# fplll/fplll

Hardware: AMD Instinct MI355X
Metric: enum nodes/sec (BKZ-60 SVP enumeration, dim-180 q-ary lattice) (higher is better)
Workload: dtype f64; 1 GPU; BASELINE configs[2]: beta=60 blocks kappa=0,1,2 of the 180-dim q-ary lattice, one Enumeration::enumerate call per step, radius min(0.99 r,1.1 GH), FastEvaluator(1); pruning=LinearPruningParams(60,30), counting_rule=fplll (after the bound test), summed in 64 bit

## Files before the change

### fplll_amd/build.py

```python
import os
import subprocess
import sys

HERE = os.path.dirname(os.path.abspath(__file__))
ROOT = os.path.dirname(HERE)
CSRC = os.path.join(HERE, "csrc")
LIBDIR = os.path.join(HERE, "lib")

HIP_SOURCES = ["enum_kernel.hip", "enum_walk.hip", "enum_kernel_cvp.hip", "enum_walk_cvp.hip", "enum_deal.hip", "enum_order.hip", "enum_host.hip", "gso_kernel.hip", "gso_sweep2.hip", "lll_kernel.hip", "lll_kernel_early.hip", "hlll_kernel.hip", "hh_blocked.hip", "hh_rows.hip", "hlll_x.hip", "lll_x.hip", "bkz_kernel.hip", "bkzs_kernel.hip", "bkz_kernel_u.hip", "bkzs_kernel_u.hip", "gso_host.hip", "pruner_volume.hip", "pruner_search.hip", "gso_util_host.hip"]
HIP_HEADERS = ["dev_mem.h", "dev_cache.h", "trace.h", "pruner_tables.h", "pruner_engine.h", "enum_device.h", "enum_order.h", "enum_wave.h", "gso_device.h", "gso_wave.h", "gso_sweep2.h", "ftx.h", "lll_wave.h", "lll_stream.h", os.path.join(ROOT, "include", "fplll_hip.h")]
HIPCC_FLAGS = [
    "--offload-arch=gfx950", "-O3", "-std=c++17",
    "-ffp-contract=off",
    "-fPIC", "-Wno-unused-value", "-Wno-inline-asm",
]


PER_FILE_FLAGS = {
    "enum_kernel.hip": ["-mllvm", "-structurizecfg-skip-uniform-regions=1", "-Xclang", "-disable-lifetime-markers"],
    "enum_walk.hip": ["-mllvm", "-structurizecfg-skip-uniform-regions=1", "-Xclang", "-disable-lifetime-markers"],
    "enum_kernel_cvp.hip": ["-mllvm", "-structurizecfg-skip-uniform-regions=1", "-Xclang", "-disable-lifetime-markers"],
    "enum_walk_cvp.hip": ["-mllvm", "-structurizecfg-skip-uniform-regions=1", "-Xclang", "-disable-lifetime-markers"],
    "bkzs_kernel.hip": ["-mllvm", "-structurizecfg-skip-uniform-regions=1", "-Xclang", "-disable-lifetime-markers"],
    "bkzs_kernel_u.hip": ["-mllvm", "-structurizecfg-skip-uniform-regions=1", "-Xclang", "-disable-lifetime-markers"],
    "bkz_kernel_u.hip": ["-mllvm", "-structurizecfg-skip-uniform-regions=1"],
    "lll_kernel.hip": ["-mllvm", "-structurizecfg-skip-uniform-regions=1"],
    "lll_kernel_early.hip": ["-mllvm", "-structurizecfg-skip-uniform-regions=1"],
    "bkz_kernel.hip": ["-mllvm", "-structurizecfg-skip-uniform-regions=1"],
    "hlll_kernel.hip": ["-mllvm", "-structurizecfg-skip-uniform-regions=1"],
    "gso_kernel.hip": ["-mllvm", "-structurizecfg-skip-uniform-regions=1"],
}


EXTRA_DEPS = {"lll_kernel_early.hip": ["lll_kernel.hip"], "enum_kernel_cvp.hip": ["enum_kernel.hip"],
              "enum_walk_cvp.hip": ["enum_walk.hip"], "bkz_kernel_u.hip": ["bkz_kernel.hip"],
              "bkzs_kernel_u.hip": ["bkzs_kernel.hip"]}


def _newer(target, deps):
    if not os.path.exists(target):
        return True
    t = os.path.getmtime(target)
    return any(os.path.exists(d) and os.path.getmtime(d) > t for d in deps)


def _run(cmd, cwd=None):
    print("[build]", " ".join(cmd), flush=True)
    subprocess.check_call(cmd, cwd=cwd)


def hipcc():
    for c in ("hipcc", "/opt/rocm/bin/hipcc"):
        try:
            subprocess.check_output([c, "--version"], stderr=subprocess.STDOUT)
            return c
        except Exception:
            continue
    raise RuntimeError("hipcc not found")


def build_hip(force=False):
    os.makedirs(LIBDIR, exist_ok=True)
    out = os.path.join(LIBDIR, "libfplll_hip.so")
    srcs = [os.path.join(CSRC, s) for s in HIP_SOURCES if os.path.exists(os.path.join(CSRC, s))]
    hdrs = [h if os.path.isabs(h) else os.path.join(CSRC, h) for h in HIP_HEADERS]
    extra = []
    if os.environ.get("FPHIP_GSO_RING"):
        extra.append("-DFPHIP_GSO_RING=" + os.environ["FPHIP_GSO_RING"])
        force = True
    objdir = os.path.join(LIBDIR, "obj")
    os.makedirs(objdir, exist_ok=True)
    objs = []
    relink = force or not os.path.exists(out)
    jobs = []
    for src in srcs:
        obj = os.path.join(objdir, os.path.basename(src) + ".o")
        objs.append(obj)
        more = [os.path.join(CSRC, x) for x in EXTRA_DEPS.get(os.path.basename(src), [])]
        if force or _newer(obj, [src, os.path.abspath(__file__)] + hdrs + more):
            jobs.append([hipcc()] + HIPCC_FLAGS + extra + PER_FILE_FLAGS.get(os.path.basename(src), []) +
                        ["-c", "-o", obj, src])
            relink = True
    if jobs:
        from concurrent.futures import ThreadPoolExecutor
        with ThreadPoolExecutor(max_workers=max(1, min(len(jobs), os.cpu_count() or 1))) as ex:
            list(ex.map(_run, jobs))
    if relink:
        _run([hipcc(), "--offload-arch=gfx950", "-fPIC", "-shared", "-pthread", "-o", out] + objs)
    return out


def build_shim(force=False):
    out = os.path.join(LIBDIR, "libfplll_hip_extenum.so")
    src = os.path.join(CSRC, "extenum_shim.cpp")
    if force or _newer(out, [src, os.path.join(ROOT, "include", "fplll_hip.h")]):
        _run(["g++", "-std=c++11", "-O2", "-fPIC", "-shared", "-o", out, src, "-L" + LIBDIR,
              "-lfplll_hip", "-Wl,-rpath,$ORIGIN", "-pthread"])
    return out


REF_HEADERS = "/root/reference"
CONDA = "/opt/conda"


def build_gso_dropin(force=False):
    out = os.path.join(LIBDIR, "libfplll_hip_gso.so")
    src = os.path.join(CSRC, "dropin", "matgso_hip.cpp")
    src2 = os.path.join(CSRC, "dropin", "mathouseholder_hip.cpp")
    hdr = os.path.join(CSRC, "dropin", "matgso_hip.h")
    hdr2 = os.path.join(CSRC, "dropin", "mathouseholder_hip.h")
    if not os.path.isdir(os.path.join(REF_HEADERS, "fplll")):
        return out if os.path.exists(out) else None
    if force or _newer(out, [src, src2, hdr, hdr2, os.path.join(ROOT, "include", "fplll_hip.h")]):
        cfg = os.path.join(LIBDIR, "obj", "fplll_cfg", "fplll")
        os.makedirs(cfg, exist_ok=True)
        with open(os.path.join(cfg, "fplll_config.h"), "w") as f:
            f.write("#ifndef FPLLL_CONFIG__H\n#define FPLLL_CONFIG__H\n#define FPLLL_MAJOR_VERSION 5\n"
                    "#define FPLLL_MINOR_VERSION 5\n#define FPLLL_MICRO_VERSION 0\n#define FPLLL_VERSION 5.5.0\n"
# ... 29 lines not shown
```

### fplll_amd/csrc/enum_host.hip

```cpp

#include <hip/hip_runtime.h>

#include <algorithm>
#include <chrono>
#include <cmath>
#include <cstdarg>
#include <cstdio>
#include <cstdlib>
#include <cstring>
#include <vector>

#include "../../include/fplll_hip.h"
#include "dev_mem.h"
#include "trace.h"
#include "enum_device.h"
#include "enum_order.h"


namespace fphip
{
template <bool MU_LDS, bool SUBS, bool DUAL>
__global__ void enum_phase_kernel(DevShared *g, HostCtl *h, TaskBuf in, TaskBuf out, int d,
                                  int Lmax, int stop, unsigned task_lo, unsigned task_hi,
                                  const unsigned *idxlist, int launch_idx, int count_nodes,
                                  unsigned budget, const double *xhi_root, double *gstk, int Tsplit,
                                  unsigned *qh, const unsigned *rcnt, unsigned rcap,
                                  unsigned long long bound_init);
template <int NQT, bool SUBS, bool DUAL>
__global__ void enum_top_kernel(DevShared *g, HostCtl *h, TopBuf in, unsigned n_in, TopBuf out_top,
                                int stop, TaskBuf out, double *xhi_root, int d, double maxdist,
                                int count_nodes, int launch_idx, double *gtop);
__global__ void task_key_kernel(TaskBuf in, unsigned n, int d, unsigned long long *keys,
                                const double *xhi_root, const unsigned *slots);
template <bool MU_LDS, bool DUAL, bool CHAIN>
__global__ void enum_walk_kernel(DevShared *g, HostCtl *h, TaskBuf in, TaskBuf out, int d, int Lmax, unsigned task_lo,
                                 unsigned task_hi, const unsigned *idxlist, int launch_idx, int count_nodes,
                                 unsigned budget, const double *xhi_root, double *gstk, int Tsplit, unsigned *qh,
                                 const unsigned *rcnt, unsigned rcap, unsigned long long bound_init);
template <bool MU_LDS, bool SUBS, bool DUAL>
__global__ void enum_phase_cvp_kernel(DevShared *g, HostCtl *h, TaskBuf in, TaskBuf out, int d, int Lmax, int stop,
                                      unsigned task_lo, unsigned task_hi, const unsigned *idxlist, int launch_idx,
                                      int count_nodes, unsigned budget, const double *xhi_root, double *gstk, int Tsplit,
                                      unsigned *qh, const unsigned *rcnt, unsigned rcap, unsigned long long bound_init);
template <bool MU_LDS, bool DUAL, bool CHAIN>
__global__ void enum_walk_cvp_kernel(DevShared *g, HostCtl *h, TaskBuf in, TaskBuf out, int d, int Lmax, unsigned task_lo,
                                     unsigned task_hi, const unsigned *idxlist, int launch_idx, int count_nodes,
                                     unsigned budget, const double *xhi_root, double *gstk, int Tsplit, unsigned *qh,
                                     const unsigned *rcnt, unsigned rcap, unsigned long long bound_init);
template <bool DUAL>
__global__ void enum_bfs_cvp_kernel(DevShared *g, double maxdist, QueueMem *qm, TaskBuf f0, TaskBuf f1, TaskBuf fin, int L0,
                                    int nlev, int floor_level, float heavy, int count_nodes, int compact_n, int shard_index,
                                    int shard_count);
size_t deal_work_bytes(unsigned n);
unsigned deal_tasks_device(hipStream_t s, const unsigned long long *keys, const double *pd, const unsigned *slot_of,
                           unsigned n, unsigned W, unsigned rank, unsigned *mine, void *work, size_t work_bytes);
size_t order_work_bytes(unsigned n);
int order_tasks_device(hipStream_t s, const DevShared *g, TaskBuf in, unsigned n, int d, const unsigned *slots,
                       unsigned *list, void *work, size_t work_bytes, int num_cus, int *sort_passes);
__global__ void task_pack_kernel(TaskBuf in, unsigned lo, unsigned n, double *rec, const double *xhi_root, int xstr);
__global__ void task_unpack_kernel(TaskBuf out, unsigned lo, unsigned n, const double *rec, double *xhi_root, int xstr,
                                   unsigned root_base);
template <bool DUAL>
__global__ void enum_bfs_kernel(DevShared *g, double maxdist, QueueMem *qm, TaskBuf f0, TaskBuf f1,
                                TaskBuf fin, int L0, int nlev, int floor_level, float heavy, int count_nodes,
                                int compact_n, int shard_index, int shard_count);
__global__ void enum_bfs_epilogue(const DevShared *g, HostCtl *h, const QueueMem *qm, unsigned rcap,
                                  unsigned *slots, double *pdc, const double *pd)
{
  __shared__ unsigned base[FPHIP_NQ + 1];
  if (threadIdx.x == 0)
  {
    unsigned tot = 0;
    for (int q = 0; q < FPHIP_NQ; ++q)
    {
      base[q] = tot;
      const unsigned c = qm->fin[q * FPHIP_QS];
      tot += c < rcap ? c : rcap;
    }
    base[FPHIP_NQ] = tot;
    h->pad[0]      = tot;
    h->pad[1]      = g->error_flags;
    __threadfence_system();
  }
  __syncthreads();
  if (slots)
    for (int q = 0; q < FPHIP_NQ; ++q)
      for (unsigned i = threadIdx.x; i < base[q + 1] - base[q]; i += blockDim.x)
      {
        slots[base[q] + i] = (unsigned)q * rcap + i;
        pdc[base[q] + i]   = pd[(size_t)q * rcap + i];
      }
}
}
using namespace fphip;

#include <mutex>
#include <vector>
namespace
{
struct PinnedBuf
{
  void *p;
  size_t bytes;
  bool busy;
};
std::mutex g_pinned_mutex;
std::vector<PinnedBuf> g_pinned;
}
#include "dev_cache.h"

void *fphip_pinned_get(size_t bytes)
{
  std::lock_guard<std::mutex> lk(g_pinned_mutex);
  PinnedBuf *best = nullptr;
  for (PinnedBuf &b : g_pinned)
    if (!b.busy && b.bytes >= bytes && (!best || b.bytes < best->bytes))
      best = &b;
  if (best)
  {
    best->busy = true;
    return best->p;
// ... 793 lines not shown
      fphip_dev_free(ctx->xhi_root, ctx->stream);
      ctx->xhi_root = nullptr;
      ctx->xhi_row  = 64;
      HIPCHK(ctx, fphip_dev_alloc((void **)&ctx->xhi_root, (size_t)ctx->cap * 192 * sizeof(double), ctx->stream));
      HIPCHK(ctx, hipMemsetAsync(ctx->xhi_root, 0, 192 * sizeof(double), ctx->stream));
      ctx->xhi_row = 192;
    }
    int cut = 64;
    for (int k = d - 1; k > 64; --k)
      if (logN[k] - logN[d] >= std::log(2048.0))
      {
        cut = k;
        break;
      }
    const int top_count = (o.shard_index == 0) ? 1 : 0;
    auto top_launch = [&](int in_idx, unsigned n_in, int stop, unsigned grid) -> int
    {
      HIPCHK(ctx, hipEventRecord(ctx->ev[0], ctx->stream));
#define FPHIP_TOP_LAUNCH(N, S_, D_)                                                                                \
  hipLaunchKernelGGL((enum_top_kernel<N, S_, D_>), dim3(grid), dim3(64), tlds, ctx->stream, ctx->g, ctx->h,          \
                     ctx->top[in_idx], n_in, ctx->top[in_idx ^ 1], stop, top_out, ctx->xhi_root, d, maxdist,        \
                     top_count, launch_idx, ctx->gtop)
      if (wide)
      {
        if (dual)
          FPHIP_TOP_LAUNCH(4, false, true);
        else if (subs)
          FPHIP_TOP_LAUNCH(4, true, false);
        else
          FPHIP_TOP_LAUNCH(4, false, false);
      }
      else if (dual)
        FPHIP_TOP_LAUNCH(2, false, true);
      else if (subs)
        FPHIP_TOP_LAUNCH(2, true, false);
      else
        FPHIP_TOP_LAUNCH(2, false, false);
#undef FPHIP_TOP_LAUNCH
      HIPCHK(ctx, hipGetLastError());
      HIPCHK(ctx, hipEventRecord(ctx->ev[1], ctx->stream));
      uint64_t nsub = 0;
      int rcw       = wait_serving(ctx, d, cb, subcb, user, &nsub);
      if (rcw != FPHIP_OK)
        return rcw;
      float tms = 0;
      HIPCHK(ctx, hipEventElapsedTime(&tms, ctx->ev[0], ctx->ev[1]));
      top_ms += tms;
      ++launch_idx;
      return FPHIP_OK;
    };
    int rct = top_launch(0, 1u, cut, 1u);
    if (rct != FPHIP_OK)
      return rct;
    if (cut > 64)
    {
      unsigned c1 = 0;
      HIPCHK(ctx, hipMemcpy(&c1, ctx->top[1].count, 4, hipMemcpyDeviceToHost));
      if (c1 > cap2)
      {
        snprintf(ctx->err, sizeof ctx->err, "more than %u top tasks: the block stays on the CPU enumerator", cap2);
        return FPHIP_UNSUPPORTED;
      }
      if (c1 > 0)
      {
        const unsigned per_cu = wide ? 4u : (unsigned)std::max<size_t>(1, (160 * 1024) / std::max<size_t>(tlds, 1));
        const unsigned grid   = std::min<unsigned>(c1, (unsigned)ctx->num_cus * std::min(per_cu, wide ? 4u : 8u));
        rct                   = top_launch(1, c1, 64, grid);
        if (rct != FPHIP_OK)
          return rct;
      }
    }
    HIPCHK(ctx, hipMemcpy(&top_tasks, ctx->buf[cur].count, 4, hipMemcpyDeviceToHost));
    if (top_tasks > top_out.cap)
    {
      snprintf(ctx->err, sizeof ctx->err,
               "more than %u surviving nodes at level 64: the block stays on the CPU enumerator", top_out.cap);
      return FPHIP_UNSUPPORTED;
    }
  }

  const int debug     = env_int("FPHIP_DEBUG", 0);
  const bool walk2    = env_int("FPHIP_WALK2", 1) != 0;
  const bool walk3    = env_int("FPHIP_WALK3", 1) != 0;
  uint64_t nsol       = 0;
  double kernel_ms    = top_ms, final_ms = 0.0;
  int launches        = 0;
  int L               = d > 64 ? 64 : d;
  unsigned C          = d > 64 ? top_tasks : 1;
  int final_tasks     = 0, final_L = d;
  const int max_split = env_int("FPHIP_MAX_SPLIT_PHASES", 6);
  double est_nodes = 0;
  for (int k = 0; k < d; ++k)
    est_nodes += std::exp(std::min(logN[k], 60.0));
  unsigned budget       = (unsigned)env_int("FPHIP_BUDGET", 1 << 22);
  const int max_rounds  = env_int("FPHIP_MAX_ROUNDS", 24);
  if (debug)
    fprintf(stderr, "[fphip] d=%d est_nodes=%.3e budget=%u\n", d, est_nodes, budget);
  unsigned long long moved_tasks = 0;
  unsigned xhi_used = d > 64 ? top_tasks : 0;
  bool in_final       = false;
  int round           = 0;
  unsigned prevC      = 0;

  bool regioned = false;
  unsigned n_slots = 0;
  bool bfs_sharded = false;
  if (use_bfs && C > 0)
  {
    FPHIP_RANGE("enum: breadth-first stage");
    const int L0        = L;
    const unsigned rcap = ctx->cap / FPHIP_NQ;
    const double want_tasks = o.target_tasks > 0 ? o.target_tasks : env_int("FPHIP_BFS_TASKS", 65536);
    float heavy = (float)std::max((double)env_int("FPHIP_BFS_HEAVY", 1024), est_nodes / want_tasks);
    int Lend = 1;
    for (int Lv = L0 - 1; Lv >= 1; --Lv)
      if (bfs_est0[Lv] <= heavy)
      {
        Lend = Lv;
        break;
      }
    Lend = std::max(Lend, std::min(L0 - 1, env_int("FPHIP_BFS_FLOOR", 4)));
    const int cnt_bfs = (o.shard_index == 0) ? 1 : 0;
    const bool shard_bfs = o.shard_count > 1 && d <= 64 && o.exchange && env_int("FPHIP_BFS_SHARD", 0) != 0;
    int n_single = 0;
    for (int Lv = L0; Lv > Lend; --Lv)
    {
      const double est_parents = (Lv == L0 ? (double)C : std::exp(std::min(logN[Lv] - logN[L0], 40.0)) * C);
      if (est_parents > env_int("FPHIP_BFS_SINGLE_MAX", 256))
        break;
      ++n_single;
    }
    HIPCHK(ctx, hipEventRecord(ctx->ev[0], ctx->stream));
    int Lv = L0, par = 0;
    int compact_n = (int)C;
    auto bfs_launch = [&](int nlev, unsigned grid, unsigned threads)
    {
      const TaskBuf &fa = ctx->buf[1 + par], &fb = ctx->buf[2 - par];
      const bool filter = shard_bfs && grid > 1u && !bfs_sharded;
      const int smode   = filter ? 1 : ((shard_bfs && !bfs_sharded) ? 2 : 0);
      const int scount  = smode ? o.shard_count * 4 + smode : 0;
      const int cnt     = (bfs_sharded || filter) ? 1 : cnt_bfs;
      if (filter)
        bfs_sharded = true;
      if (cvp)
        hipLaunchKernelGGL((enum_bfs_cvp_kernel<false>), dim3(grid), dim3(threads), 0, ctx->stream, ctx->g, maxdist,
                           ctx->qm, fa, fb, ctx->buf[0], Lv, nlev, Lend, heavy, cnt, compact_n, o.shard_index, scount);
      else if (dual)
        hipLaunchKernelGGL((enum_bfs_kernel<true>), dim3(grid), dim3(threads), 0, ctx->stream, ctx->g, maxdist,
                           ctx->qm, fa, fb, ctx->buf[0], Lv, nlev, Lend, heavy, cnt, compact_n, o.shard_index, scount);
      else
        hipLaunchKernelGGL((enum_bfs_kernel<false>), dim3(grid), dim3(threads), 0, ctx->stream, ctx->g, maxdist,
                           ctx->qm, fa, fb, ctx->buf[0], Lv, nlev, Lend, heavy, cnt, compact_n, o.shard_index, scount);
      Lv -= nlev;
      par ^= nlev & 1;
      compact_n = -1;
      ++launches;
    };
    if (n_single > 0)
      bfs_launch(n_single, 1u, 1024u);
    const unsigned bgrid = std::max(32u, ((unsigned)ctx->num_cus * (unsigned)env_int("FPHIP_BFS_WG_PER_CU", 1)) / 32u * 32u);
    while (Lv > Lend)
      bfs_launch(1, bgrid, 256u);
    const bool want_slots = (o.shard_count > 1 && !bfs_sharded) || ordered;
    hipLaunchKernelGGL(enum_bfs_epilogue, dim3(1), dim3(1024), 0, ctx->stream, ctx->g, ctx->h, ctx->qm, rcap,
                       want_slots ? ctx->slots : nullptr, want_slots ? ctx->pdc : nullptr, ctx->buf[0].pd);
    HIPCHK(ctx, hipGetLastError());
// ... 192 lines not shown
        task_x.resize((size_t)span * 64);
        task_level.resize(span);
        HIPCHK(ctx, hipMemcpy(task_x.data(), ctx->buf[cur].x, (size_t)span * 64 * sizeof(double), hipMemcpyDeviceToHost));
        HIPCHK(ctx, hipMemcpy(task_level.data(), ctx->buf[cur].level, (size_t)span * sizeof(int), hipMemcpyDeviceToHost));
        std::vector<unsigned> ranks((size_t)C * d);
        for (unsigned i = 0; i < C; ++i)
          order_vector(d, mut, rdiag, &task_x[(size_t)where[i] * 64], task_level[where[i]], &ranks[(size_t)i * d], nullptr);
        std::vector<unsigned> perm(C);
        for (unsigned i = 0; i < C; ++i)
          perm[i] = i;
        std::stable_sort(perm.begin(), perm.end(), [&](unsigned a, unsigned b)
                         { return order_before(d, &ranks[(size_t)a * d], &ranks[(size_t)b * d]); });
        for (unsigned i = 0; i < C; ++i)
          order_host[i] = where[perm[i]];
        HIPCHK(ctx, hipMemcpy(ctx->idxlist, order_host.data(), (size_t)C * 4, hipMemcpyHostToDevice));
        order_passes = -1;
      }
      else
        HIPCHK(ctx, hipMemcpy(order_host.data(), ctx->idxlist, (size_t)C * 4, hipMemcpyDeviceToHost));
      idxl = ctx->idxlist;
      if (debug)
        fprintf(stderr, "[fphip] ordered: %u tasks sorted %s (%d radix passes)\n", C,
                order_passes < 0 ? "on the host" : "on the device", order_passes);
      unsigned first = 1024;
      double grow    = 8.0;
      if (const char *ws = getenv("FPHIP_ORDER_WINDOWS"))
        if (*ws)
        {
          double g2 = 0.0;
          const int got = sscanf(ws, "%u,%lf", &first, &g2);
          if (got >= 2 && g2 >= 1.0)
            grow = g2;
        }
      cuts.push_back(0u);
      double wsz = (double)first;
      while (cuts.back() < C)
      {
        const bool last = first == 0u || cuts.size() > 128u || launch_idx + (int)cuts.size() + 1 >= FPHIP_MAX_LAUNCHES;
        const double nxtcut = last ? (double)C : std::min((double)C, (double)cuts.back() + std::max(1.0, wsz));
        cuts.push_back((unsigned)nxtcut);
        wsz *= grow;
      }
    }
    const int count_nodes = (in_final || o.shard_index == 0) ? 1 : 0;
    HIPCHK(ctx, hipMemsetAsync(ctx->buf[nxt].count, 0, 4, ctx->stream));

    const int nchunk = order_now ? (int)cuts.size() - 1 : chunks;
    for (int ch = 0; ch < nchunk; ++ch)
    {
      unsigned lo = order_now ? cuts[ch] : (unsigned)(((unsigned long long)n_list * ch) / chunks);
      unsigned hi = order_now ? cuts[ch + 1] : (unsigned)(((unsigned long long)n_list * (ch + 1)) / chunks);
      if (hi <= lo && !(in_final && o.exchange))
        continue;
      unsigned mine = hi - lo;
      unsigned grid = std::min<unsigned>((mine + wpb - 1) / wpb,
                                         (unsigned)(ctx->num_cus * blocks_per_cu));
      if (grid == 0)
        grid = 1;
      if (launch_idx >= FPHIP_MAX_LAUNCHES)
        return fail(ctx, "too many launches");
      if (hi > lo)
      {
        FPHIP_RANGE(in_final ? "enum: walk launch" : "enum: split launch");
        HIPCHK(ctx, hipEventRecord(ctx->ev[0], ctx->stream));
        const unsigned bud =
            (in_final && round < max_rounds && (!subs || env_int("FPHIP_SUBS_DONATE", 1) != 0) && !ordered) ? budget : 0u;
#define FPHIP_LAUNCH(M, S, D) FPHIP_LAUNCH_K(enum_phase_kernel, M, S, D)
#define FPHIP_LAUNCH_K(KERNEL, M, S, D)                                                             \
  hipLaunchKernelGGL((KERNEL<M, S, D>), dim3(grid), dim3(wpb * 64), lds, ctx->stream, ctx->g, \
                     ctx->h, ctx->buf[cur], ctx->buf[nxt], d, L, stop, lo, hi, idxl, launch_idx,     \
                     count_nodes, bud, ctx->xhi_root, ctx->gstk, Ts, &ctx->qm->head[launch_idx][0],          \
                     (regioned && !shard_now && !order_now) ? &ctx->qm->fin[0] : (const unsigned *)nullptr, ctx->cap / FPHIP_NQ, \
                     (unsigned long long)__atomic_load_n(&ctx->h->bound_bits, __ATOMIC_ACQUIRE))
#define FPHIP_LAUNCH2_K(M, D, C) FPHIP_LAUNCH2_KK(enum_walk_kernel, M, D, C)
#define FPHIP_LAUNCH2_KK(KERNEL, M, D, C)                                                            \
  hipLaunchKernelGGL((KERNEL<M, D, C>), dim3(grid), dim3(wpb * 64), lds, ctx->stream, ctx->g, \
                     ctx->h, ctx->buf[cur], ctx->buf[nxt], d, L, lo, hi, idxl, launch_idx,           \
                     count_nodes, bud, ctx->xhi_root, ctx->gstk, Ts, &ctx->qm->head[launch_idx][0],  \
                     (regioned && !shard_now && !order_now) ? &ctx->qm->fin[0] : (const unsigned *)nullptr, ctx->cap / FPHIP_NQ, \
                     (unsigned long long)__atomic_load_n(&ctx->h->bound_bits, __ATOMIC_ACQUIRE))
#define FPHIP_LAUNCH2(M, D)                                                                          \
  do                                                                                                 \
  {                                                                                                  \
    if (walk3)                                                                                       \
      FPHIP_LAUNCH2_K(M, D, true);                                                                   \
    else                                                                                             \
      FPHIP_LAUNCH2_K(M, D, false);                                                                  \
  } while (0)
        if (cvp)
        {
          if (in_final && walk2 && walk3)
          {
            if (mu_lds)
              FPHIP_LAUNCH2_KK(enum_walk_cvp_kernel, true, false, true);
            else
              FPHIP_LAUNCH2_KK(enum_walk_cvp_kernel, false, false, true);
          }
          else if (in_final && walk2)
          {
            if (mu_lds)
              FPHIP_LAUNCH2_KK(enum_walk_cvp_kernel, true, false, false);
            else
              FPHIP_LAUNCH2_KK(enum_walk_cvp_kernel, false, false, false);
          }
          else if (mu_lds)
            FPHIP_LAUNCH_K(enum_phase_cvp_kernel, true, false, false);
          else
            FPHIP_LAUNCH_K(enum_phase_cvp_kernel, false, false, false);
        }
        else if (in_final && !subs && walk2)
        {
          if (dual && mu_lds)
            FPHIP_LAUNCH2(true, true);
          else if (dual)
            FPHIP_LAUNCH2(false, true);
          else if (mu_lds)
            FPHIP_LAUNCH2(true, false);
          else
            FPHIP_LAUNCH2(false, false);
        }
        else if (dual && mu_lds)
          FPHIP_LAUNCH(true, false, true);
        else if (dual)
          FPHIP_LAUNCH(false, false, true);
        else if (mu_lds && !subs)
          FPHIP_LAUNCH(true, false, false);
        else if (!mu_lds && !subs)
          FPHIP_LAUNCH(false, false, false);
        else if (mu_lds)
          FPHIP_LAUNCH(true, true, false);
        else
          FPHIP_LAUNCH(false, true, false);
#undef FPHIP_LAUNCH
#undef FPHIP_LAUNCH_K
#undef FPHIP_LAUNCH2
#undef FPHIP_LAUNCH2_K
#undef FPHIP_LAUNCH2_KK
        HIPCHK(ctx, hipGetLastError());
        HIPCHK(ctx, hipEventRecord(ctx->ev[1], ctx->stream));
        ++launch_idx;
        int rc = wait_serving(ctx, d, cb_dev, subcb, user_dev, &nsol);
        if (rc != FPHIP_OK)
          return rc;
        float ms = 0.f;
        HIPCHK(ctx, hipEventElapsedTime(&ms, ctx->ev[0], ctx->ev[1]));
        kernel_ms += ms;
        if (in_final)
          final_ms += ms;
        if (debug)
        {
          unsigned long long it = 0;
          hipMemcpy(&it, &ctx->g->iters, 8, hipMemcpyDeviceToHost);
          fprintf(stderr,
                  "[fphip s%d] launch %d %s tasks [%u,%u) L=%d stop=%d budget=%u grid=%u wpb=%d lds=%zu "
                  "-> %.3f ms, iters so far %llu\n",
                  o.shard_index, launch_idx - 1, in_final ? "walk" : "split", lo, hi, L, stop,
                  in_final ? budget : 0u, grid, wpb, lds, ms, it);
        }
      }
      if (order_now)
      {
        ++windows;
        if (hi < n_list)
        {
          double xr[64];
          int lv = 0;
          unsigned fr[64];
// ... 142 lines not shown
```

### fplll_amd/csrc/enum_walk.hip

```cpp

#include <hip/hip_runtime.h>
#include <stdint.h>

#include "enum_device.h"
#include "enum_wave.h"

#ifndef FPHIP_CVP
#define FPHIP_CVP 0
#endif
#if FPHIP_CVP
#define FPHIP_WALK_KERNEL enum_walk_cvp_kernel
#else
#define FPHIP_WALK_KERNEL enum_walk_kernel
#endif

namespace fphip
{

#define ST_I(s) ((s)&0x7f)
#define ST_N(s) (((s) >> 8) & 0x7f)
#define ST_MARK 0x7f64
#define ST_IS_SLOW(s) (((s)&0x7fff) == ST_MARK)
#define ST_IW(s) ((int)((unsigned)(s) >> 17))

__device__ __forceinline__ int zig_of(int i, bool down)
{
  const int hh = (i + 1) >> 1;
  const int z  = (i & 1) ? hh : -hh;
  return down ? -z : z;
}

__device__ __forceinline__ v2u r_issue(const double *tab, unsigned off)
{
  v2u q;
  asm volatile("s_load_dwordx2 %0, %1, %2" : "=s"(q) : "s"(tab), "s"(off));
  return q;
}
__device__ __forceinline__ void rp_wait(v2u &q) { asm volatile("s_waitcnt lgkmcnt(0)" : "+s"(q)); }
__device__ __forceinline__ double rp_r2(const v2u &q) { return __hiloint2double((int)q.y, (int)q.x); }

template <bool MU_LDS, bool DUAL, bool CHAIN>
__global__ void __launch_bounds__(FPHIP_MAX_BLOCK) __attribute__((amdgpu_waves_per_eu(8, 8)))
    FPHIP_WALK_KERNEL(DevShared *__restrict__ g, HostCtl *__restrict__ h, TaskBuf in, TaskBuf out,
                     int d, int Lmax, unsigned task_lo, unsigned task_hi,
                     const unsigned *__restrict__ idxlist, int launch_idx, int count_nodes,
                     unsigned budget, const double *__restrict__ xhi_root, double *__restrict__ gstk,
                     int Tsplit, unsigned *__restrict__ qh, const unsigned *__restrict__ rcnt, unsigned rcap,
                     unsigned long long bound_init)
{
  constexpr bool CVP = FPHIP_CVP != 0;
  extern __shared__ __attribute__((aligned(16))) double smem[];
  const int lane = threadIdx.x & 63;
  const int wave = __builtin_amdgcn_readfirstlane((int)(threadIdx.x >> 6));
  constexpr unsigned MUROW8 = FPHIP_MUROW * 8u;
  const unsigned lane8 = (unsigned)lane << 3;
  const int triL = (Lmax * (Lmax + 1)) >> 1;
  const double *mu_s;
  const int nw     = (int)(blockDim.x >> 6);
  const int Ts     = min(Tsplit, Lmax + 1);
  const int Tsm1   = Ts - 1;
  const int ldsRow = tri_off(Ts);
  const int ldsWave = ldsRow + FPHIP_STACK_PAD;
  double *stk;
  if constexpr (MU_LDS)
  {
    double *mu_l = smem;
    stk          = smem + triL + wave * ldsWave;
    const int nmu = (Lmax * (Lmax - 1)) >> 1;
    for (int i = threadIdx.x; i < nmu; i += blockDim.x)
      mu_l[i] = g->mu_tri[i];
    mu_s = mu_l;
  }
  else
  {
    mu_s = &g->mu_sq[0][0];
    stk  = smem + wave * ldsWave;
  }
  if constexpr (MU_LDS)
    __syncthreads();
  const __amdgpu_buffer_rsrc_t mu_b = mu_rsrc(&g->mu_sq[0][0], (unsigned)sizeof(g->mu_sq));
  char *stk_top      = (char *)stk + (((unsigned)ldsRow << 3) + lane8);
  double *gst = gstk + (size_t)(blockIdx.x * nw + wave) * (size_t)(triL - ldsRow + 1) - ldsRow;
  const double *rptab = &g->mu_sq[0][64];
  double zz = (lane & 15) == 0 ? 0.0 : (double)zig_of(lane - (lane >> 4), false);
  FPHIP_IN_VGPR(zz);

  unsigned long long mbits =
      rfl_u64(min(bound_init, __hip_atomic_load(&g->bound_bits, __ATOMIC_RELAXED, __HIP_MEMORY_SCOPE_AGENT)));
  double maxdist   = __longlong_as_double((long long)mbits);
  double maxdist_v = maxdist;
  FPHIP_IN_VGPR(maxdist_v);

  double cs = 0.0, x0s = 0.0, pds = 0.0;
  int st = 0;
  unsigned long long cnt = 0;
  unsigned cnt32         = 0;
  unsigned iter          = 0;
  constexpr int RF = 24;
  int left               = RF - 1;

#define FPHIP_REFRESH_BOUND(from_host, bchg)                                                      \
  do                                                                                              \
  {                                                                                               \
    unsigned long long nb_;                                                                       \
    if (from_host)                                                                                \
    {                                                                                             \
      nb_ = load_sys_u64(&h->bound_bits);                                                         \
      if (nb_ < mbits && lane == 0)                                                               \
        atomicMin(&g->bound_bits, nb_);                                                           \
      FPHIP_JOIN();                                                                               \
    }                                                                                             \
    else                                                                                          \
    {                                                                                             \
      nb_ = __hip_atomic_load(&g->bound_bits, __ATOMIC_RELAXED, __HIP_MEMORY_SCOPE_AGENT);        \
    }                                                                                             \
    nb_ = rfl_u64(nb_);                                                                           \
    if (nb_ < mbits)                                                                              \
    {                                                                                             \
      mbits   = nb_;                                                                              \
      maxdist = __longlong_as_double((long long)mbits);                                           \
      maxdist_v = maxdist;                                                                        \
      FPHIP_IN_VGPR(maxdist_v);                                                                   \
      bchg = true;                                                                                \
    }                                                                                             \
  } while (0)

  unsigned q = (unsigned)__builtin_amdgcn_readfirstlane((int)((blockIdx.x * nw + wave) % FPHIP_NQ));
  const unsigned nlist = task_hi - task_lo;
  for (;;)
  {
    unsigned t = 0, cq = 0;
    bool have = false;
    for (;;)
    {
      if (lane == 0)
        t = atomicAdd(&qh[q * FPHIP_QS], 1u);
      t  = (unsigned)__builtin_amdgcn_readfirstlane((int)t);
      cq = rcnt ? min((unsigned)__builtin_amdgcn_readfirstlane((int)rcnt[q * FPHIP_QS]), rcap)
                : (nlist > q ? (nlist - q + FPHIP_NQ - 1u) / FPHIP_NQ : 0u);
      if (t < cq)
      {
        have = true;
        break;
      }
      bool any = false;
#pragma unroll
      for (unsigned hf = 0; hf < FPHIP_NQ / 64; ++hf)
      {
        const unsigned qq = (q + 1u + hf * 64u + (unsigned)lane) % FPHIP_NQ;
        const unsigned hd = __hip_atomic_load(&qh[qq * FPHIP_QS], __ATOMIC_RELAXED, __HIP_MEMORY_SCOPE_AGENT);
        const unsigned cn = rcnt ? min(rcnt[qq * FPHIP_QS], rcap)
                                 : (nlist > qq ? (nlist - qq + FPHIP_NQ - 1u) / FPHIP_NQ : 0u);
        const unsigned long long m = __builtin_amdgcn_ballot_w64(hd < cn);
        if (m != 0ull)
        {
          q   = (q + 1u + hf * 64u + (unsigned)__builtin_ctzll(m)) % FPHIP_NQ;
          any = true;
          break;
        }
      }
      if (!any)
        break;
    }
    if (!have)
    {
      if (budget != 0u && lane == 0)
        __hip_atomic_store(&g->drain[launch_idx], 1u, __ATOMIC_RELAXED, __HIP_MEMORY_SCOPE_AGENT);
      FPHIP_JOIN();
      break;
    }
    const unsigned long long pos = (unsigned long long)task_lo + q + (unsigned long long)t * FPHIP_NQ;
    const unsigned long long ti =
        rcnt ? (unsigned long long)q * rcap + (cq - 1u - t)
             : (idxlist ? (unsigned long long)(unsigned)__builtin_amdgcn_readfirstlane((int)idxlist[pos]) : pos);
    const int Lt      = __builtin_amdgcn_readfirstlane(in.level[ti]);
    const int rid     = __builtin_amdgcn_readfirstlane(in.root[ti]);
    double xpre = 0.0, col0 = 0.0;
    if constexpr (!CHAIN)
    {
      const int tl = here_lane(lane);
      xpre         = in.x[ti * 64 + tl];
      col0         = in.col[ti * 64 + tl];
    }
    const double pd0  = in.pd[ti];
    int donate        = 1 << 20;
    const unsigned iter0 = iter;
    {
      bool bchg = false;
      FPHIP_REFRESH_BOUND((t & 63u) == 0u, bchg);
    }

    int k     = Lt;
    double S  = col0;
    if constexpr (CHAIN)
      S = in.col[ti * 64 + here_lane(lane)];
    double nd = pd0;
    bool zc = __builtin_amdgcn_ballot_w64(pd0 != 0.0) == 0ull;
    if constexpr (CVP)
      zc = false;
    unsigned long long P = 0ull, B = 0ull;
    if constexpr (!CHAIN)
      st = (lane == (Lt & 63)) ? ST_MARK : st;

    auto xs_now = [&]() -> double
    {
      const int idx = (lane == 0) ? 0 : (ST_IS_SLOW(st) ? ST_IW(st) : ST_I(st));
      return x0s + (double)zig_of(idx, !(cs >= x0s));
    };
    auto path_x = [&](int klo) -> double
    {
      if constexpr (!CHAIN)
        return (lane < Lt) ? xs_now() : xpre;
      else
      {
        const int tl = here_lane(lane);
        double Sr    = in.col[ti * 64 + tl];
        double xr    = (lane >= Lt) ? in.x[ti * 64 + tl] : 0.0;
        for (int l = Lt - 1; l >= klo; --l)
        {
          const double c = rl_f64(Sr, l);
          double x;
          if ((B >> l) & 1ull)
          {
            const int s_    = rl_i32(st, l);
            const double x0 = rl_f64(x0s, l);
            x = x0 + (double)zig_of(ST_IS_SLOW(s_) ? ST_IW(s_) : ST_I(s_), !(rl_f64(cs, l) >= x0));
          }
          else
          {
            x = rint(c);
            const double al = x - c;
            if (fabs(al) == 0.5 && ((al < 0.0) == (c > 0.0)))
              x = x - (al + al);
          }
          xr = (lane == l) ? x : xr;
          const double ml = ld_row(mu_b, (unsigned)l * MUROW8, lane8);
          Sr = Sr - (DUAL ? x - c : x) * ml;
        }
        if (lane == 0)
          atomicAdd(&g->replays, 1u);
        FPHIP_JOIN();
        return xr;
      }
    };

    auto report = [&](double dist, double xleaf, bool &bchg)
    {
      unsigned long long idx = 0;
      if (lane == 0)
        idx = atomicAdd(&g->sol_head, 1ull);
      idx = rfl_u64(idx);
      for (unsigned spin = 0; idx >= load_sys_u64(&h->consumed) + FPHIP_RING_CAP; ++spin)
      {
        __builtin_amdgcn_s_sleep(64);
        if (spin > (1u << 24))
        {
          if (lane == 0)
            atomicOr(&g->error_flags, FPHIP_ERR_RING_TIMEOUT);
          break;
        }
      }
      SolRec *r  = &h->ring[idx % FPHIP_RING_CAP];
      const double xf = (CHAIN && lane == 0) ? xleaf : path_x(1);
      const int rl = here_lane(lane);
      r->x[rl]   = (lane < d) ? xf : 0.0;
      {
        const int xstr = d > 64 ? 64 * ((d - 1) >> 6) : 64;
#pragma unroll
        for (int qq = 1; qq < 4; ++qq)
          r->x[64 * qq + rl] = (64 * qq + lane < d) ? xhi_root[(size_t)rid * xstr + 64 * (qq - 1) + rl] : 0.0;
      }
      if (lane == 0)
      {
        const int z = here_lane(0);
        r->dist     = dist;
        r->kind     = z;
        r->offset   = z;
      }
      __threadfence_system();
      if (lane == 0)
        __hip_atomic_store(&r->seq, idx + 1, __ATOMIC_RELEASE, __HIP_MEMORY_SCOPE_SYSTEM);
      for (unsigned spin = 0; load_sys_u64(&h->consumed) <= idx; ++spin)
      {
        __builtin_amdgcn_s_sleep(32);
        if (spin > (1u << 24))
        {
          if (lane == 0)
            atomicOr(&g->error_flags, FPHIP_ERR_RING_TIMEOUT);
          break;
        }
      }
      FPHIP_REFRESH_BOUND(true, bchg);
    };

    auto reprune = [&](int klo)
    {
      int s_           = st;
      const bool act   = lane >= klo && lane < Lt && (!CHAIN || ((B >> lane) & 1ull) != 0ull) && !ST_IS_SLOW(s_);
      const double r_l = g->rdiag[lane];
      const double b_l = g->pruning[lane] * maxdist;
      const int cur    = ST_I(s_);
      const bool down  = !(cs >= x0s);
      int n            = ST_N(s_);
      for (;;)
      {
        const int j      = n - 1;
        const double xj  = x0s + (double)zig_of(j, down);
        const double aj  = xj - cs;
        const double ndj = pds + aj * aj * r_l;
        const bool fail  = act && j > cur && !(ndj <= b_l);
        if (__builtin_amdgcn_ballot_w64(fail) == 0ull)
          break;
        if (fail)
          n -= 1;
      }
      s_ = (s_ & ~(0x7f << 8)) | (n << 8);
      st = act ? s_ : st;
      if constexpr (CHAIN)
        P &= ~__builtin_amdgcn_ballot_w64(act && cur + 1 >= n);
      FPHIP_JOIN();
    };

    enum : int { EV_EMIT = 1, EV_DONE = 3, EV_REFRESH = 6, EV_SPECIAL = 7, EV_FAIL = 8, EV_SLOWSTEP = 10 };
    unsigned elo  = (unsigned)donate;
    unsigned erng = 0x7fffffffu;
    bool buffer_full = false;
    bool resume_step = false;
    double par = 0.0, mk = 0.0;
    double xk = 0.0, a = 0.0;
    int kc = 0;
    double mk1 = 0.0, c1 = 0.0, x1 = 0.0, a1 = 0.0;
#define FPHIP_PUSH(in_lds, kk, lds8)                                            \
  if (__builtin_expect(in_lds, 1))                                              \
    *(double *)(stk_top - (lds8)) = S;                                          \
  else                                                                          \
  {                                                                             \
    int kt = (kk);                                                              \
    asm volatile("" : "+s"(kt));                                                \
    const unsigned gk8 = ((unsigned)(kt * (kt - 1)) << 2) + lane8;              \
    *(double *)((char *)gst + ((lane < kt) ? gk8 : (unsigned)triL << 3)) = S;   \
  }
#define FPHIP_LOAD_PAR_MK()                                                     \
  do                                                                            \
  {                                                                             \
    const unsigned k8_  = (unsigned)k << 3;                                     \
    const unsigned cl8_ = min(lane8, k8_ - 8u);                                 \
    if (k + 1 < Ts)                                                             \
      par = *(const double *)(stk_top - tri8(k + 2));                           \
    else                                                                        \
      par = ld_off(gst, tri8(k + 1) + cl8_);                                    \
    if constexpr (MU_LDS)                                                       \
      mk = ld_off(mu_s, tri8(k) + cl8_);                                        \
    else                                                                        \
      mk = ld_row(mu_b, (unsigned)k * MUROW8, lane8);                           \
  } while (0)
    for (;;)
    {
      int ev;
      bool at_step = resume_step;
      resume_step  = false;
      unsigned spec_t = zc ? 0u : (elo >= 2u ? elo - 2u : 0u);
      spec_t          = (unsigned)__builtin_amdgcn_readfirstlane((int)spec_t);
      int ka = lane_addr(k);
      for (;;)
      {
        if (!at_step)
        {
          kc = k - 1;
          for (;;)
          {
            asm volatile("" : "+s"(kc));
            const unsigned kc8 = (unsigned)kc << 3;
            v4i q1             = rp_issue2(rptab, (unsigned)kc * MUROW8);
            if constexpr (MU_LDS)
              mk1 = ld_off(mu_s, tri8(kc) + min(lane8, kc8 - 8u));
            else
              mk1 = ld_row(mu_b, (unsigned)kc * MUROW8, lane8);
            ka -= 4;
            c1 = bp_f64(S, ka);
            x1 = rint(c1);
            a1 = x1 - c1;
            const double aj  = a1 + zz;
            rp_wait(q1);
            const double bnd = rp_p(q1) * maxdist_v;
            const double ndj = nd + aj * aj * rp_r(q1);
            const unsigned long long m = __builtin_amdgcn_ballot_w64(ndj <= bnd);
            if (m == 0ull)
            {
              ev = EV_FAIL;
              FPHIP_EXIT();
              break;
            }
            if ((unsigned)(kc - 1) >= spec_t)
            {
              ev = EV_SPECIAL;
              FPHIP_EXIT();
              break;
            }
            int c = __builtin_popcountll(m);
            asm("" : "+s"(c));
            if (c == 64)
            {
              ev = EV_SPECIAL;
              FPHIP_EXIT();
              break;
            }
            const unsigned long long me = lane_bit(kc);
            if (CHAIN && c == 4)
            {
              B &= ~me;
              cnt32 = add_bit(me, cnt32);
              nd    = row_bcast0_f64(ndj);
              S     = S - (DUAL ? a1 : x1) * mk1;
              --kc;
              continue;
            }
            if (__builtin_amdgcn_ballot_w64(fabs(a1) == 0.5) != 0ull)
            {
              asm volatile("");
              const bool fix = (a1 < 0.0) == (c1 > 0.0);
              x1             = fix ? x1 - (a1 + a1) : x1;
              a1 = __hiloint2double(__double2hiint(a1) ^ (fix ? (int)0x80000000 : 0), __double2loint(a1));
            }
            FPHIP_PUSH(kc < Ts - 1, kc + 1, tri8(kc + 2));
            if constexpr (CHAIN)
            {
              P |= me;
              B |= me;
            }
            cs    = sel_f64(me, c1, cs);
            x0s   = sel_f64(me, x1, x0s);
            pds   = sel_f64(me, nd, pds);
            st    = wl_i32((c - 3) << 8, kc, st);
            cnt32 = add_bit(me, cnt32);
            nd    = row_bcast0_f64(ndj);
            S     = S - (DUAL ? a1 : x1) * mk1;
            --kc;
          }
          k = kc + 1;
          ka += 4;
          if (ev != EV_FAIL)
            break;
        }
        at_step = false;
        int tk;
        if constexpr (CHAIN)
        {
          if (__builtin_expect(P == 0ull, 0))
          {
            ev = EV_DONE;
            break;
          }
          k  = __builtin_ctzll(P);
          ka = lane_addr(k);
          tk = rl_i32(st, k) + 1;
        }
        else
        {
          for (;;)
          {
            tk = rl_i32(st, k) + 1;
            if (__builtin_expect((tk & 0x7f) < ((tk >> 8) & 0x7f), 1))
              break;
            ++k;
            ka += 4;
          }
        }
        if (__builtin_expect((tk & 0x7f) >= 64, 0))
        {
          ev = EV_SLOWSTEP;
          break;
        }
        if (__builtin_expect(--left < 0, 0))
        {
          ev = EV_REFRESH;
          break;
        }
        if constexpr (CHAIN)
          if ((tk & 0x7f) + 1 >= ((tk >> 8) & 0x7f))
            P &= ~lane_bit(k);
        {
          v2u qk = r_issue(rptab, (unsigned)k * MUROW8);
          if (__builtin_expect(k < Tsm1, 1))
            par = *(const double *)(stk_top - tri8(k + 2));
          else
          {
            int kt = k;
            asm volatile("" : "+s"(kt));
            par = ld_off(gst, tri8(kt + 1) + min(lane8, ((unsigned)kt << 3) - 8u));
          }
          if constexpr (MU_LDS)
            mk = ld_off(mu_s, tri8(k) + min(lane8, ((unsigned)k << 3) - 8u));
          else
            mk = ld_row(mu_b, (unsigned)k * MUROW8, lane8);
          int zi;
          {
            const int ii = tk & 0x7f;
            const int hh = (ii + 1) >> 1;
            zi           = (ii & 1) ? hh : -hh;
            asm("" : "+s"(zi));
          }
          const double zd  = (double)zi;
          const double x0  = bp_f64(x0s, ka);
          const double ck  = bp_f64(cs, ka);
          const double pk  = bp_f64(pds, ka);
          st               = wl_i32(tk, k, st);
          cnt32            = add_bit(lane_bit(k), cnt32);
          const double sgd = __hiloint2double((ck >= x0) ? 0x3ff00000 : (int)0xbff00000, 0);
          xk               = __builtin_fma(zd, sgd, x0);
          a                = xk - ck;
          rp_wait(qk);
          nd = pk + a * a * rp_r2(qk);
          S  = par - (DUAL ? a : xk) * mk;
        }
      }
      FPHIP_OPAQUE(ev);
      if (ev == EV_SPECIAL)
      {
        if ((unsigned)(k - elo) <= erng)
          ev = EV_EMIT;
        else if (k == 1)
        {
          bool bchg       = false;
          const double c0 = rl_f64(S, 0);
          double x = rint(c0), al = x - c0;
          if (fabs(al) == 0.5 && ((al < 0.0) == (c0 > 0.0)))
          {
            x  = x - (al + al);
            al = -al;
          }
          int dx         = (c0 >= x) ? 1 : -1;
          bool zig       = __builtin_amdgcn_ballot_w64(nd != 0.0) != 0ull;
          if constexpr (CVP)
            zig = true;
          const double r0 = g->rdiag[0], p0 = g->pruning[0];
          for (;;)
          {
            const double ndc = nd + al * al * r0;
            if (__builtin_amdgcn_ballot_w64(ndc <= p0 * maxdist) == 0ull)
              break;
            cnt += (lane == 0) ? 1ull : 0ull;
            if (CVP || __builtin_amdgcn_ballot_w64(ndc > 0.0) != 0ull)
            {
              if constexpr (!CHAIN)
              {
                x0s = (lane == 0) ? x : x0s;
                cs  = (lane == 0) ? x : cs;
              }
              report(ndc, x, bchg);
              FPHIP_JOIN();
            }
            if (zig)
            {
              x += (double)dx;
              dx = (dx > 0 ? -1 : 1) - dx;
            }
            else
              x += 1.0;
            al = x - c0;
          }
          if (bchg)
            reprune(1);
          resume_step = true;
          continue;
        }
        else
        {
          const bool nz = __builtin_amdgcn_ballot_w64(nd != 0.0) != 0ull;
          if (zc && nz)
            zc = false;
          kc              = k - 1;
          const double rk = g->rdiag[kc], pk = g->pruning[kc];
          if constexpr (MU_LDS)
            mk1 = ld_off(mu_s, tri8(kc) + min(lane8, ((unsigned)kc << 3) - 8u));
          else
            mk1 = ld_row(mu_b, (unsigned)kc * MUROW8, lane8);
          c1 = rl_f64(S, kc);
          x1 = rint(c1);
          a1 = x1 - c1;
          if (fabs(a1) == 0.5 && ((a1 < 0.0) == (c1 > 0.0)))
          {
            x1 = x1 - (a1 + a1);
            a1 = -a1;
          }
          const double nd1 = nd + a1 * a1 * rk;
          if (__builtin_amdgcn_ballot_w64(nd1 <= pk * maxdist) == 0ull)
          {
            resume_step = true;
            continue;
          }
          FPHIP_PUSH(k < Ts, k, tri8(k + 1));
          if constexpr (CHAIN)
          {
            P |= lane_bit(kc);
            B |= lane_bit(kc);
          }
          cs  = (lane == kc) ? c1 : cs;
          x0s = (lane == kc) ? x1 : x0s;
          pds = (lane == kc) ? nd : pds;
          st  = (lane == kc) ? ST_MARK : st;
          cnt += (lane == kc) ? 1ull : 0ull;
          nd  = nd1;
          S   = S - (DUAL ? a1 : x1) * mk1;
          k   = kc;
          FPHIP_JOIN();
          continue;
        }
      }
      if (CHAIN && ev == EV_DONE)
        break;
      if (ev == EV_SLOWSTEP)
      {
        if (!CHAIN && k >= Lt)
          break;
        const int stk_  = rl_i32(st, k);
        const int cur   = ST_IW(stk_);
        const double x0 = rl_f64(x0s, k), ck = rl_f64(cs, k), pk = rl_f64(pds, k);
        const double rk = g->rdiag[k], pr = g->pruning[k];
        bool grow       = __builtin_amdgcn_ballot_w64(pk != 0.0) == 0ull;
        if constexpr (CVP)
          grow = false;
        const bool down = __builtin_amdgcn_ballot_w64(ck >= x0) == 0ull;
        const int nxt   = grow ? (cur == 0 ? 1 : cur + 2) : cur + 1;
        xk              = x0 + (double)zig_of(nxt, down);
        a               = xk - ck;
        const double ndn = pk + a * a * rk;
        const bool ok    = nxt < 32760 && __builtin_amdgcn_ballot_w64(ndn <= pr * maxdist) != 0ull;
        if (!ok)
        {
          if constexpr (CHAIN)
            P &= ~lane_bit(k);
          else
          {
            st = (lane == k) ? 0 : st;
            ++k;
          }
          resume_step = true;
          FPHIP_JOIN();
          continue;
        }
        st = (lane == k) ? (ST_MARK | (nxt << 17)) : st;
        cnt += (lane == k) ? 1ull : 0ull;
        FPHIP_LOAD_PAR_MK();
        nd = ndn;
        S  = par - (DUAL ? a : xk) * mk;
        FPHIP_JOIN();
        continue;
      }
      if (ev == EV_EMIT)
      {
        unsigned oi = 0;
        if (lane == 0)
          oi = atomicAdd(out.count, 1u);
        oi = (unsigned)__builtin_amdgcn_readfirstlane((int)oi);
        if (oi < out.cap)
        {
          const int el                              = here_lane(lane);
          out.col[(unsigned long long)oi * 64 + el] = S;
          const double xf                           = path_x(k);
          out.x[(unsigned long long)oi * 64 + el]   = xf;
          if (lane == 0)
          {
            out.pd[oi]    = nd;
            out.level[oi] = k;
            out.root[oi]  = rid;
          }
          FPHIP_JOIN();
        }
        else
        {
          if (lane == 0)
            atomicOr(&g->error_flags, FPHIP_FLAG_TASK_OVERFLOW);
          FPHIP_JOIN();
          buffer_full = true;
          donate      = 1 << 20;
          elo         = 1u << 20;
          erng        = 0u;
          continue;
        }
      }
      else if (ev == EV_REFRESH)
      {
        cnt += cnt32;
        cnt32 = 0u;
        iter += 64u;
        left = RF - 1;
        bool bchg = false;
        FPHIP_REFRESH_BOUND((iter & 16383u) == 0u, bchg);
        if (bchg)
          reprune(k);
        const unsigned titer = iter - iter0;
        if (budget != 0u && titer >= 64u && !buffer_full)
        {
          const unsigned dr = (unsigned)__builtin_amdgcn_readfirstlane((int)__hip_atomic_load(
              &g->drain[launch_idx], __ATOMIC_RELAXED, __HIP_MEMORY_SCOPE_AGENT));
          if (dr != 0u || titer >= budget)
          {
            donate = min(donate, k + 1);
            elo    = (unsigned)donate;
          }
        }
        FPHIP_JOIN();
      }
      resume_step = true;
    }
#undef FPHIP_PUSH
#undef FPHIP_LOAD_PAR_MK
    cnt += cnt32;
    cnt32 = 0u;
  }
#undef FPHIP_REFRESH_BOUND

  if (count_nodes && cnt != 0)
    atomicAdd(&g->nodes[lane], cnt);
  if (lane == 0)
    atomicAdd(&g->iters, (unsigned long long)iter);
}

#define FPHIP_INST(M, D, C)                                                                             \
  template __global__ void FPHIP_WALK_KERNEL<M, D, C>(DevShared *, HostCtl *, TaskBuf, TaskBuf, int, int, \
                                                  unsigned, unsigned, const unsigned *, int, int,       \
                                                  unsigned, const double *, double *, int, unsigned *,   \
                                                  const unsigned *, unsigned, unsigned long long);
FPHIP_INST(true, false, false)
FPHIP_INST(false, false, false)
#if !FPHIP_CVP
FPHIP_INST(true, true, false)
FPHIP_INST(false, true, false)
#endif
FPHIP_INST(true, false, true)
FPHIP_INST(false, false, true)
#if !FPHIP_CVP
FPHIP_INST(true, true, true)
FPHIP_INST(false, true, true)
#endif
#undef FPHIP_INST

}
```

Measured before the change: 26.17 billion nodes/s.

## Add walk4 enum kernel that precomputes sibling pair on fresh descent

Adds a new walk kernel variant, built as enum_walk4.hip and enabled by default through FPHIP_WALK4. When the walk first descends into a level, it also computes the second zig-zag sibling (x1±1) and records its partial distance and center sum in a pending mask Q. When that level is revisited, the pending sibling is consumed directly from the saved state, skipping the usual zig-zag step recomputation. This adds more mask bookkeeping and reprune logic for pending siblings, and raises register pressure and risk to node-count correctness.

```diff
diff --git a/fplll_amd/build.py b/fplll_amd/build.py
--- a/fplll_amd/build.py
+++ b/fplll_amd/build.py
@@ -7,7 +7,7 @@
 CSRC = os.path.join(HERE, "csrc")
 LIBDIR = os.path.join(HERE, "lib")
 
-HIP_SOURCES = ["enum_kernel.hip", "enum_walk.hip", "enum_kernel_cvp.hip", "enum_walk_cvp.hip", "enum_deal.hip", "enum_order.hip", "enum_host.hip", "gso_kernel.hip", "gso_sweep2.hip", "lll_kernel.hip", "lll_kernel_early.hip", "hlll_kernel.hip", "hh_blocked.hip", "hh_rows.hip", "hlll_x.hip", "lll_x.hip", "bkz_kernel.hip", "bkzs_kernel.hip", "bkz_kernel_u.hip", "bkzs_kernel_u.hip", "gso_host.hip", "pruner_volume.hip", "pruner_search.hip", "gso_util_host.hip"]
+HIP_SOURCES = ["enum_kernel.hip", "enum_walk.hip", "enum_kernel_cvp.hip", "enum_walk_cvp.hip", "enum_walk4.hip", "enum_deal.hip", "enum_order.hip", "enum_host.hip", "gso_kernel.hip", "gso_sweep2.hip", "lll_kernel.hip", "lll_kernel_early.hip", "hlll_kernel.hip", "hh_blocked.hip", "hh_rows.hip", "hlll_x.hip", "lll_x.hip", "bkz_kernel.hip", "bkzs_kernel.hip", "bkz_kernel_u.hip", "bkzs_kernel_u.hip", "gso_host.hip", "pruner_volume.hip", "pruner_search.hip", "gso_util_host.hip"]
 HIP_HEADERS = ["dev_mem.h", "dev_cache.h", "trace.h", "pruner_tables.h", "pruner_engine.h", "enum_device.h", "enum_order.h", "enum_wave.h", "gso_device.h", "gso_wave.h", "gso_sweep2.h", "ftx.h", "lll_wave.h", "lll_stream.h", os.path.join(ROOT, "include", "fplll_hip.h")]
 HIPCC_FLAGS = [
     "--offload-arch=gfx950", "-O3", "-std=c++17",
@@ -21,6 +21,7 @@
     "enum_walk.hip": ["-mllvm", "-structurizecfg-skip-uniform-regions=1", "-Xclang", "-disable-lifetime-markers"],
     "enum_kernel_cvp.hip": ["-mllvm", "-structurizecfg-skip-uniform-regions=1", "-Xclang", "-disable-lifetime-markers"],
     "enum_walk_cvp.hip": ["-mllvm", "-structurizecfg-skip-uniform-regions=1", "-Xclang", "-disable-lifetime-markers"],
+    "enum_walk4.hip": ["-mllvm", "-structurizecfg-skip-uniform-regions=1", "-Xclang", "-disable-lifetime-markers"],
     "bkzs_kernel.hip": ["-mllvm", "-structurizecfg-skip-uniform-regions=1", "-Xclang", "-disable-lifetime-markers"],
     "bkzs_kernel_u.hip": ["-mllvm", "-structurizecfg-skip-uniform-regions=1", "-Xclang", "-disable-lifetime-markers"],
     "bkz_kernel_u.hip": ["-mllvm", "-structurizecfg-skip-uniform-regions=1"],
@@ -33,7 +34,7 @@
 
 
 EXTRA_DEPS = {"lll_kernel_early.hip": ["lll_kernel.hip"], "enum_kernel_cvp.hip": ["enum_kernel.hip"],
-              "enum_walk_cvp.hip": ["enum_walk.hip"], "bkz_kernel_u.hip": ["bkz_kernel.hip"],
+              "enum_walk_cvp.hip": ["enum_walk.hip"], "enum_walk4.hip": ["enum_walk.hip"], "bkz_kernel_u.hip": ["bkz_kernel.hip"],
               "bkzs_kernel_u.hip": ["bkzs_kernel.hip"]}
 
 
diff --git a/fplll_amd/csrc/enum_host.hip b/fplll_amd/csrc/enum_host.hip
--- a/fplll_amd/csrc/enum_host.hip
+++ b/fplll_amd/csrc/enum_host.hip
@@ -37,6 +37,11 @@
                                  unsigned task_hi, const unsigned *idxlist, int launch_idx, int count_nodes,
                                  unsigned budget, const double *xhi_root, double *gstk, int Tsplit, unsigned *qh,
                                  const unsigned *rcnt, unsigned rcap, unsigned long long bound_init);
+template <bool MU_LDS, bool DUAL>
+__global__ void enum_walk4_kernel(DevShared *g, HostCtl *h, TaskBuf in, TaskBuf out, int d, int Lmax, unsigned task_lo,
+                                  unsigned task_hi, const unsigned *idxlist, int launch_idx, int count_nodes,
+                                  unsigned budget, const double *xhi_root, double *gstk, int Tsplit, unsigned *qh,
+                                  const unsigned *rcnt, unsigned rcap, unsigned long long bound_init);
 template <bool MU_LDS, bool SUBS, bool DUAL>
 __global__ void enum_phase_cvp_kernel(DevShared *g, HostCtl *h, TaskBuf in, TaskBuf out, int d, int Lmax, int stop,
                                       unsigned task_lo, unsigned task_hi, const unsigned *idxlist, int launch_idx,
@@ -996,6 +1001,7 @@
   const int debug     = env_int("FPHIP_DEBUG", 0);
   const bool walk2    = env_int("FPHIP_WALK2", 1) != 0;
   const bool walk3    = env_int("FPHIP_WALK3", 1) != 0;
+  const bool walk4    = env_int("FPHIP_WALK4", 1) != 0;
   uint64_t nsol       = 0;
   double kernel_ms    = top_ms, final_ms = 0.0;
   int launches        = 0;
@@ -1354,7 +1360,13 @@
 #define FPHIP_LAUNCH2(M, D)                                                                          \
   do                                                                                                 \
   {                                                                                                  \
-    if (walk3)                                                                                       \
+    if (walk3 && walk4)                                                                              \
+      hipLaunchKernelGGL((enum_walk4_kernel<M, D>), dim3(grid), dim3(wpb * 64), lds, ctx->stream, ctx->g, \
+                         ctx->h, ctx->buf[cur], ctx->buf[nxt], d, L, lo, hi, idxl, launch_idx,       \
+                         count_nodes, bud, ctx->xhi_root, ctx->gstk, Ts, &ctx->qm->head[launch_idx][0], \
+                         (regioned && !shard_now && !order_now) ? &ctx->qm->fin[0] : (const unsigned *)nullptr, ctx->cap / FPHIP_NQ, \
+                         (unsigned long long)__atomic_load_n(&ctx->h->bound_bits, __ATOMIC_ACQUIRE)); \
+    else if (walk3)                                                                                  \
       FPHIP_LAUNCH2_K(M, D, true);                                                                   \
     else                                                                                             \
       FPHIP_LAUNCH2_K(M, D, false);                                                                  \
diff --git a/fplll_amd/csrc/enum_walk.hip b/fplll_amd/csrc/enum_walk.hip
--- a/fplll_amd/csrc/enum_walk.hip
+++ b/fplll_amd/csrc/enum_walk.hip
@@ -12,6 +12,16 @@
 #define FPHIP_WALK_KERNEL enum_walk_cvp_kernel
 #else
 #define FPHIP_WALK_KERNEL enum_walk_kernel
+#endif
+#ifndef FPHIP_WALK4
+#define FPHIP_WALK4 0
+#endif
+#if FPHIP_WALK4
+#undef FPHIP_WALK_KERNEL
+#define FPHIP_WALK_KERNEL enum_walk4_kernel
+#define FPHIP_W4_PAIR 1
+#else
+#define FPHIP_W4_PAIR 0
 #endif
 
 namespace fphip
@@ -39,7 +49,11 @@
 __device__ __forceinline__ void rp_wait(v2u &q) { asm volatile("s_waitcnt lgkmcnt(0)" : "+s"(q)); }
 __device__ __forceinline__ double rp_r2(const v2u &q) { return __hiloint2double((int)q.y, (int)q.x); }
 
+#if FPHIP_WALK4
+template <bool MU_LDS, bool DUAL>
+#else
 template <bool MU_LDS, bool DUAL, bool CHAIN>
+#endif
 __global__ void __launch_bounds__(FPHIP_MAX_BLOCK) __attribute__((amdgpu_waves_per_eu(8, 8)))
     FPHIP_WALK_KERNEL(DevShared *__restrict__ g, HostCtl *__restrict__ h, TaskBuf in, TaskBuf out,
                      int d, int Lmax, unsigned task_lo, unsigned task_hi,
@@ -49,6 +63,9 @@
                      unsigned long long bound_init)
 {
   constexpr bool CVP = FPHIP_CVP != 0;
+#if FPHIP_WALK4
+  constexpr bool CHAIN = true;
+#endif
   extern __shared__ __attribute__((aligned(16))) double smem[];
   const int lane = threadIdx.x & 63;
   const int wave = __builtin_amdgcn_readfirstlane((int)(threadIdx.x >> 6));
@@ -199,6 +216,9 @@
     if constexpr (CVP)
       zc = false;
     unsigned long long P = 0ull, B = 0ull;
+#if FPHIP_W4_PAIR
+    unsigned long long Q = 0ull;
+#endif
     if constexpr (!CHAIN)
       st = (lane == (Lt & 63)) ? ST_MARK : st;
 
@@ -220,6 +240,11 @@
         {
           const double c = rl_f64(Sr, l);
           double x;
+#if FPHIP_W4_PAIR
+          if ((B >> l) & (Q >> l) & 1ull)
+            x = rl_f64(x0s, l);
+          else
+#endif
           if ((B >> l) & 1ull)
           {
             const int s_    = rl_i32(st, l);
@@ -296,7 +321,11 @@
     auto reprune = [&](int klo)
     {
       int s_           = st;
+#if FPHIP_W4_PAIR
+      const bool act   = lane >= klo && lane < Lt && (((B & ~Q) >> lane) & 1ull) != 0ull && !ST_IS_SLOW(s_);
+#else
       const bool act   = lane >= klo && lane < Lt && (!CHAIN || ((B >> lane) & 1ull) != 0ull) && !ST_IS_SLOW(s_);
+#endif
       const double r_l = g->rdiag[lane];
       const double b_l = g->pruning[lane] * maxdist;
       const int cur    = ST_I(s_);
@@ -318,6 +347,14 @@
       st = act ? s_ : st;
       if constexpr (CHAIN)
         P &= ~__builtin_amdgcn_ballot_w64(act && cur + 1 >= n);
+#if FPHIP_W4_PAIR
+      {
+        const bool pend = lane >= klo && lane < Lt && (((P & Q) >> lane) & 1ull) != 0ull;
+        const unsigned long long gone = __builtin_amdgcn_ballot_w64(pend && !(pds <= b_l));
+        P &= ~gone;
+        Q &= ~gone;
+      }
+#endif
       FPHIP_JOIN();
     };
 
@@ -422,6 +459,29 @@
               x1             = fix ? x1 - (a1 + a1) : x1;
               a1 = __hiloint2double(__double2hiint(a1) ^ (fix ? (int)0x80000000 : 0), __double2loint(a1));
             }
+#if FPHIP_W4_PAIR
+            if (c == 5)
+            {
+              const double sd  = __hiloint2double((c1 >= x1) ? 0x3ff00000 : (int)0xbff00000, 0);
+              const double x2  = x1 + sd;
+              const double a2  = x2 - c1;
+              const double nd2 = nd + a2 * a2 * rp_r(q1);
+              const double S1  = S - (DUAL ? a1 : x1) * mk1;
+              S                = S - (DUAL ? a2 : x2) * mk1;
+              FPHIP_PUSH(kc < Ts - 1, kc + 1, tri8(kc + 2));
+              P |= me;
+              Q |= me;
+              B &= ~me;
+              x0s = sel_f64(me, x2, x0s);
+              pds = sel_f64(me, nd2, pds);
+              cnt32 = add_bit(me, cnt32);
+              nd    = row_bcast0_f64(ndj);
+              S  = S1;
+              --kc;
+              continue;
+            }
+            Q &= ~me;
+#endif
             FPHIP_PUSH(kc < Ts - 1, kc + 1, tri8(kc + 2));
             if constexpr (CHAIN)
             {
@@ -453,6 +513,30 @@
           }
           k  = __builtin_ctzll(P);
           ka = lane_addr(k);
+#if FPHIP_W4_PAIR
+          if ((Q >> k) & 1ull)
+          {
+            if (__builtin_expect(--left < 0, 0))
+            {
+              ev = EV_REFRESH;
+              break;
+            }
+            const unsigned long long me = lane_bit(k);
+            P &= ~me;
+            B |= me;
+            if (__builtin_expect(k < Tsm1, 1))
+              S = *(const double *)(stk_top - tri8(k + 2));
+            else
+            {
+              int kt = k;
+              asm volatile("" : "+s"(kt));
+              S = ld_off(gst, tri8(kt + 1) + min(lane8, ((unsigned)kt << 3) - 8u));
+            }
+            nd = bp_f64(pds, ka);
+            cnt32 = add_bit(me, cnt32);
+            continue;
+          }
+#endif
           tk = rl_i32(st, k) + 1;
         }
         else
@@ -595,6 +679,9 @@
             P |= lane_bit(kc);
             B |= lane_bit(kc);
           }
+#if FPHIP_W4_PAIR
+          Q &= ~lane_bit(kc);
+#endif
           cs  = (lane == kc) ? c1 : cs;
           x0s = (lane == kc) ? x1 : x0s;
           pds = (lane == kc) ? nd : pds;
@@ -717,6 +804,18 @@
     atomicAdd(&g->iters, (unsigned long long)iter);
 }
 
+#if FPHIP_WALK4
+#define FPHIP_INST4(M, D)                                                                            \
+  template __global__ void FPHIP_WALK_KERNEL<M, D>(DevShared *, HostCtl *, TaskBuf, TaskBuf, int, int, \
+                                                  unsigned, unsigned, const unsigned *, int, int,       \
+                                                  unsigned, const double *, double *, int, unsigned *,   \
+                                                  const unsigned *, unsigned, unsigned long long);
+FPHIP_INST4(true, false)
+FPHIP_INST4(false, false)
+FPHIP_INST4(true, true)
+FPHIP_INST4(false, true)
+#undef FPHIP_INST4
+#else
 #define FPHIP_INST(M, D, C)                                                                             \
   template __global__ void FPHIP_WALK_KERNEL<M, D, C>(DevShared *, HostCtl *, TaskBuf, TaskBuf, int, int, \
                                                   unsigned, unsigned, const unsigned *, int, int,       \
@@ -735,5 +834,6 @@
 FPHIP_INST(false, true, true)
 #endif
 #undef FPHIP_INST
+#endif
 
 }
diff --git a/fplll_amd/csrc/enum_walk4.hip b/fplll_amd/csrc/enum_walk4.hip
--- /dev/null
+++ b/fplll_amd/csrc/enum_walk4.hip
@@ -0,0 +1,2 @@
+#define FPHIP_WALK4 1
+#include "enum_walk.hip"
```

After: 28.77 billion nodes/s (median of 6 runs). 1.1x the previous value.
